# LariWa/Fractal-Image-Compression

Hardware: AMD Instinct MI355X
Metric: range-block matches/sec (8x8 R, 16x16 D, 8 iso) (higher is better)
Workload: dtype u8

## Files before the change

### fractal-image-compression_amd/csrc/fic_capi.cpp

```cpp
#include "fic_internal.h"

namespace ficd {

thread_local std::string g_err;
thread_local int g_err_code = 0;

int fail(int code, const char* fmt, ...)
{
    char buf[512];
    va_list ap;
    va_start(ap, fmt);
    vsnprintf(buf, sizeof(buf), fmt, ap);
    va_end(ap);
    g_err = buf;
    g_err_code = code;
    return code;
}

int check_device(int device)
{
    int ndev = fic_device_count();
    if (ndev <= 0 || device < 0 || device >= ndev) return fail(FIC_E_NO_DEVICE, "no HIP device %d (this library has no CPU path)", device);
    HIP_TRY(hipSetDevice(device));
    return FIC_OK;
// ... 357 lines not shown
{
    const FicGeom& g = c->g;
    const QShape q = q_shape(g);
    const int tsz = 64 * g.NR;
    const int cpr = fic_q_cols_per_range(g.B, g.n_iso);
    const int ct_begin = tile0 * tsz * cpr / 32, ct_end = tile1 * tsz * cpr / 32;
    int nchunks = c->opt_chunks;
    if (nchunks <= 0) {
        const long long base_wg = (long long)((ct_end - ct_begin + q.CT - 1) / q.CT) * g.planes;
        const long long resident = 256LL * fic_q_resident(g.B);
        auto ceil_div = [](long long a, long long b) { return (a + b - 1) / b; };
        const long long min_tiles = g.n_iso == 8 ? 30 : 14;
        long long fill = base_wg < resident ? ceil_div(2 * resident, base_wg) : 1;
        if (fill > q.ndtiles / min_tiles) fill = q.ndtiles / min_tiles;
        long long bal = ceil_div(8 * resident, base_wg);
        if (bal > q.ndtiles / 1024) bal = q.ndtiles / 1024;
        const long long nc = fill > bal ? fill : bal;
        nchunks = (int)(nc < 1 ? 1 : nc);
    }
    if (nchunks > q.ndtiles) nchunks = q.ndtiles;
    int tiles_per_chunk = (q.ndtiles + nchunks - 1) / nchunks;
    tiles_per_chunk = (tiles_per_chunk + q.unroll - 1) / q.unroll * q.unroll;
    nchunks = (q.ndtiles + tiles_per_chunk - 1) / tiles_per_chunk;
    if (fused_fin && !c->q_fin) {
        const size_t nfin = (size_t)g.planes * (q.nct_alloc / q.CT + 1);
        HIP_TRY(hipMalloc((void**)&c->q_fin, nfin * sizeof(unsigned int)));
        HIP_TRY(hipMemsetAsync(c->q_fin, 0, nfin * sizeof(unsigned int), s));
    }
    if (fic_launch_sweep_q(c->b, c->q_pool, c->q_flat, c->q_rng, c->q_rngC, c->q_E, c->q_thg, g, ct_begin, ct_end, q.ndtiles, q.ndtiles_alloc,
                           q.nct_alloc, tiles_per_chunk, nchunks, s, c->q_stats, c->opt_noflag, fused_fin ? &c->o : nullptr, c->q_fin,
                           r_begin, r_count))
        return fail(FIC_E_HIP, "k_sweep_q launch failed");
    *nchunks_out = nchunks;
    c->last_tiles_per_chunk = tiles_per_chunk;
    return FIC_OK;
}

}

extern "C" {

#ifdef FIC_BUILD_XCHECK
const char* fic_version(void) { return "fic-hip 0.3 (gfx950, +xcheck sweeps)"; }
#else
const char* fic_version(void) { return "fic-hip 0.3 (gfx950)"; }
#endif
const char* fic_last_error(void) { return g_err.c_str(); }
int fic_last_error_code(void) { return g_err_code; }

int fic_device_count(void)
{
    int n = 0;
    if (hipGetDeviceCount(&n) != hipSuccess) return 0;
    return n;
// ... 153 lines not shown
        const char* env = getenv("FIC_SWEEP");
        if (env && env[0] >= '2' && env[0] <= '6' && env[1] == '\0' && g.full) {
            const int want = env[0] - '0';
            kind = want == 5 ? valu : want;
        }
    }
    if (kind >= 2 && !g.full) return fail(FIC_E_ARGUMENT, "fast sweep needs full search (wK == Dw == Dh)");
#ifndef FIC_BUILD_XCHECK
    if (kind == 3 || kind == 4) return fail(FIC_E_ARGUMENT, "sweep %d (cross-check kernel) is not in this build (FIC_BUILD_XCHECK=0)", kind);
#endif
    if (kind == 5 && !d4_available(g)) return fail(FIC_E_ARGUMENT, "sweep 5 (k_sweep_d4) needs full search, n_iso = 8 and B = 8");
    if (kind == 6 && g.Nd >= (1 << 24)) return fail(FIC_E_ARGUMENT, "sweep 6 (k_sweep_q) needs a pool of fewer than 2^24 blocks");
    const int tsz = 64 * g.NR;
    const int tile0 = range_begin / tsz;
    const int tile1 = (range_begin + range_count + tsz - 1) / tsz;
    const int ntiles = tile1 - tile0;
    int nchunks = 1;
    int rc = FIC_OK;
    bool fused_prep = false;
    if (kind == 6) {
        const QShape q = q_shape(g);
        fused_prep = fic_q_prep_fused(g, q.ndtiles_alloc, tile1 * (64 * g.NR) / 64 - tile0 * (64 * g.NR) / 64) != 0;
    }
    if (!fused_prep && fic_launch_scale(c->b.gray, c->b.scaled, g, s)) return fail(FIC_E_HIP, "k_scale launch failed");
    if (kind == 6) {
        rc = q_prep(c, tile0, tile1, s);
    } else {
        if (fic_launch_pool(c->b.scaled, c->b.pool_pix, c->b.pool_st, c->b.pool_var, c->b.pool_s64, g, s))
            return fail(FIC_E_HIP, "k_pool launch failed");
        if (kind != 5 && !c->b.rng_pix) {
            int rca = dev_alloc(&c->b.rng_pix, (size_t)g.planes * g.Nr_pad * g.n_iso * g.DW);
            if (rca) return rca;
        }
        if (fic_launch_range(c->b.gray, c->b.rng_pix, c->b.rng_st, g, s, kind == 5 ? 0 : 1)) return fail(FIC_E_HIP, "k_range launch failed");
        HIP_TRY(hipMemset2DAsync(c->b.key + (size_t)tile0 * tsz, (size_t)g.Nr_pad * sizeof(unsigned long long), 0xFF,
                                 (size_t)ntiles * tsz * sizeof(unsigned long long), (size_t)g.planes, s));
        if (kind == 5) rc = d4_prep(c, s);
        else if (kind >= 3) rc = matrix_core_prep(c, kind, s);
    }
    if (rc == FIC_OK) rc = time_begin(c, s);
    if (rc == FIC_OK) {
        if (kind == 1) {
            if (fic_launch_sweep_generic(c->b, g, range_begin, range_count, s)) rc = fail(FIC_E_HIP, "k_sweep_generic launch failed");
        } else if (kind == 6) {
            rc = q_sweep(c, tile0, tile1, s, &nchunks, fused_prep, range_begin, range_count);
        } else if (kind == 5) {
            rc = d4_sweep(c, tile0, tile1 - tile0, s, &nchunks);
        } else if (kind >= 3) {
            rc = matrix_core_sweep(c, kind, tile0, tile1, s, &nchunks);
        } else {
            rc = valu_sweep(c, tile0, tile1 - tile0, s, &nchunks);
        }
    }
    if (rc == FIC_OK) rc = time_end(c, s);
    if (rc != FIC_OK) return rc;
    c->last_chunks = nchunks;
    c->last_kind = kind;
    c->last_fused = fused_prep ? 1 : 0;
    if (!fused_prep &&
        fic_launch_finalize(c->b, c->o, g, range_begin, range_count, s, (kind == 5 || kind == 6) ? 1 : 0)) return fail(FIC_E_HIP, "k_finalize launch failed");
    c->encoded_any = true;
    return FIC_OK;
}

int fic_ctx_sync(fic_ctx* c)
{
    if (!c) return fail(FIC_E_ARGUMENT, "fic_ctx_sync: null context");
    HIP_TRY(hipSetDevice(c->device));
    HIP_TRY(hipStreamSynchronize(c->last_stream));
    return FIC_OK;
}

int fic_ctx_get_results_host(fic_ctx* c, int32_t* idx_local, float* a, float* b, int32_t* iso, int32_t* qrows,
                             int32_t* idx_global, float* err)
{
    if (!c) return fail(FIC_E_ARGUMENT, "fic_ctx_get_results_host: null context");
    if (!c->encoded_any) return fail(FIC_E_STATE, "fic_ctx_get_results_host: nothing encoded yet");
    HIP_TRY(hipSetDevice(c->device));
    HIP_TRY(hipStreamSynchronize(c->last_stream));
    size_t n = (size_t)c->g.planes * c->g.Nr;
    if (n > (size_t)65536) {
        if (idx_local) HIP_TRY(hipMemcpy(idx_local, c->o.idx_local, n * 4, hipMemcpyDeviceToHost));
// ... 281 lines not shown
```

### fractal-image-compression_amd/csrc/fic_q.hip

```cpp
#include <hip/hip_runtime.h>
#include <stdint.h>
#include <math.h>
#include <string.h>
#include <stdlib.h>
#include <type_traits>
#include "fic_device.h"
#include "fic_launch.h"
#include "fic_devfn.h"

typedef int v4i __attribute__((ext_vector_type(4)));
typedef float v16f __attribute__((ext_vector_type(16)));
typedef _Float16 f16x8 __attribute__((ext_vector_type(8)));

#define FIC_Q_LEVEL 0.99999237060546875f
#define FIC_Q_TAU_ALL 3.0e38f
#define FIC_Q_TAU_NONE (-1.0f)
#define FIC_Q_LMIN 0.26f
#define FIC_Q_ECOEF 7.0e-4f
#define FIC_Q_EABS 1.6e-5f
#define FIC_Q_QCAP 1280
#define FIC_Q_QFLUSH 256

#ifndef FIC_Q_CTW_B8
#define FIC_Q_CTW_B8 4
// ... 62 lines not shown
        const int i = t / B, ry = t % B;
        const int d = dtile * 32 + i;
        uint32_t w[B / 4];
#pragma unroll
        for (int q = 0; q < B / 4; q++) w[q] = 0u;
        if (d < g.Nd) {
            const int c = d % g.Dw, r = d / g.Dw;
            const size_t so = (size_t)plane * g.Ws * g.Hs + (size_t)(r * g.abstand + ry) * g.Ws + c * g.abstand;
            if constexpr (!FUSE) {
                __builtin_memcpy(w, scaled_in + so, B);
            } else {
                const int ys = r * g.abstand + ry, xs0 = c * g.abstand;
                const uint8_t* im = gray + (size_t)plane * g.W * g.H + (size_t)(2 * ys) * g.W + 2 * xs0;
                uint32_t top[B / 2], bot[B / 2];
                __builtin_memcpy(top, im, 2 * B);
                __builtin_memcpy(bot, im + g.W, 2 * B);
#pragma unroll
                for (int x = 0; x < B; x++) {
                    const uint32_t t2 = top[x >> 1] >> (16 * (x & 1)), b2 = bot[x >> 1] >> (16 * (x & 1));
                    const int tap4 = (2 * (xs0 + x) + 1 >= g.H) ? 128 : (int)((b2 >> 8) & 0xffu);
                    const int m = (int)(t2 & 0xffu) + (int)((t2 >> 8) & 0xffu) + (int)(b2 & 0xffu) + tap4;
                    w[x >> 2] |= (uint32_t)(m / 4) << (8 * (x & 3));
                }
                __builtin_memcpy(scaled_out + so, w, B);
            }
        }
        uint32_t sum = 0, sq = 0;
#pragma unroll
        for (int q = 0; q < B / 4; q++) {
            sum = __builtin_amdgcn_sad_u8(w[q], 0u, sum);
            sq = __builtin_amdgcn_udot4(w[q], w[q], sq, false);
            *(uint32_t*)&pix[i][ry * B + 4 * q] = w[q];
        }
        s_sum[i][ry] = (int)sum;
        s_sq[i][ry] = (int)sq;
    }
    __syncthreads();
    for (int t = threadIdx.x; t < 32 * n / 16; t += 256) {
        const int i = t / (n / 16), q = t % (n / 16);
        const int d = dtile * 32 + i;
        if (d < g.Nd) *(uint4*)(pool_pix + ((size_t)plane * g.Nd_pad + d) * n + 16 * q) = *(const uint4*)&pix[i][16 * q];
    }
    if (threadIdx.x < 32) {
        const int i = threadIdx.x, d = dtile * 32 + i;
        int S = 0, Q = 0;
        for (int t = 0; t < B; t++) { S += s_sum[i][t]; Q += s_sq[i][t]; }
        const int m = S >> g.lgn;
// ... 30 lines not shown
            for (int u = 0; u < 8; u++) px[u] = (int)(((u < 4 ? pw.x : pw.y) >> (8 * (u & 3))) & 0xffu);
#pragma unroll
            for (int u = 0; u < 4; u++)
                v[u] = f16_pair(__fmul_rn((float)(px[2 * u] - dM), w), __fmul_rn((float)(px[2 * u + 1] - dM), w));
        } else {
            const bool odd = m >= NK / 2;
            const int p0 = 16 * (odd ? m - NK / 2 : m) + 8 * h;
            const uint2 pw = *(const uint2*)&pix[i][p0], qw = *(const uint2*)&pix[i][n - 8 - p0];
            float f[8];
#pragma unroll
            for (int u = 0; u < 8; u++) {
                const int a = (int)(((u < 4 ? pw.x : pw.y) >> (8 * (u & 3))) & 0xffu);
                const int b = (int)(((u < 4 ? qw.y : qw.x) >> (8 * (3 - (u & 3)))) & 0xffu);
                f[u] = __fmul_rn(__fmul_rn((float)(odd ? a - b : a + b - 2 * dM), w), 0.5f);
            }
#pragma unroll
            for (int u = 0; u < 4; u++) v[u] = f16_pair(f[2 * u], f[2 * u + 1]);
        }
        poolQ[((size_t)plane * ndtiles_alloc + dtile) * NK * 64 + t] = v;
    }
    if (threadIdx.x == 0) dflat[(size_t)plane * ndtiles_alloc + dtile] = s_nonflat ? 0u : 1u;
}
template <int B>
__global__ __launch_bounds__(256) void k_pool_q(const uint8_t* __restrict__ scaled, uint8_t* __restrict__ pool_pix,
                                                FicDomStat* __restrict__ pool_st, uint32_t* __restrict__ pool_var,
                                                double* __restrict__ pool_s64, v4i* __restrict__ poolQ,
                                                uint32_t* __restrict__ dflat, FicGeom g, int ndtiles_alloc, int folded, int shape16)
{
    pool_q_body<B, false>(blockIdx.x, blockIdx.y, scaled, nullptr, nullptr, pool_pix, pool_st, pool_var, pool_s64, poolQ, dflat, g,
                          ndtiles_alloc, folded, shape16);
}

__global__ __launch_bounds__(256) void k_range_q(const uint8_t* __restrict__ gray, FicRngStat* __restrict__ rng_st,
                                                 float* __restrict__ rngE, unsigned long long* __restrict__ key,
                                                 uint32_t* __restrict__ theta_g, v4i* __restrict__ rngQ,
                                                 uint32_t* __restrict__ rngC, FicGeom g, int nct_alloc, int grp0, int mode,
                                                 int staged, int shape16)
{
    __shared__ __attribute__((aligned(16))) uint8_t blk[64 * (256 + 4)];
    extern __shared__ __attribute__((aligned(16))) uint8_t cpy[];
    __shared__ int s_rM[64];
    const int plane = blockIdx.y;
    const int grp = grp0 + blockIdx.x;
    const int B = g.B, n = g.n, DW = g.DW, NK = n / 16;
    const int lgB = B == 4 ? 2 : (B == 8 ? 3 : 4);
    const int stride = n + 4;
    const int j0 = grp * 64;
    const uint8_t* img = gray + (size_t)plane * g.W * g.H;
    for (int i = threadIdx.x; i < 64 * DW; i += 256) {
        const int l = i / DW, wd = i % DW;
        const int j = j0 + l;
        uint32_t v = 0;
        if (j < g.Nr) {
// ... 330 lines not shown
}
__device__ __forceinline__ float max16_sum(const v16f& a, const v16f& b)
{
    float v[16];
#pragma unroll
    for (int e = 0; e < 16; e++) v[e] = fabsf(a[e]) + fabsf(b[e]);
    const float m0 = fmaxf(fmaxf(v[0], v[1]), v[2]), m1 = fmaxf(fmaxf(v[3], v[4]), v[5]), m2 = fmaxf(fmaxf(v[6], v[7]), v[8]);
    const float m3 = fmaxf(fmaxf(v[9], v[10]), v[11]), m4 = fmaxf(fmaxf(v[12], v[13]), v[14]);
    return fmaxf(fmaxf(fmaxf(m0, m1), m2), fmaxf(fmaxf(m3, m4), v[15]));
}

template <int MODE> struct QMode {
    static constexpr int CSHIFT = (MODE == 0 || MODE == 3) ? 0 : ((MODE == 1 || MODE == 4) ? 3 : 2);
    static constexpr int NISO = (MODE == 0 || MODE == 3) ? 1 : 8;
    static constexpr bool RGB = MODE == 3 || MODE == 4;
};
template <int MODE> __device__ __forceinline__ int q_col_iso(int c) { return MODE == 2 ? (c == 0 ? 0 : (c == 1 ? 1 : (c == 2 ? 4 : 6))) : c; }

__device__ __forceinline__ void q_key_min(unsigned long long* keyp, unsigned long long best)
{
    if (best < __hip_atomic_load(keyp, __ATOMIC_RELAXED, __HIP_MEMORY_SCOPE_AGENT)) atomicMin(keyp, best);
}

template <int NK, int MODE>
__device__ __forceinline__ void q_flush(const QArgs& A, const uint32_t* myq, int qn, int plane, int ctw0, int lane)
{
    constexpr int NISO = QMode<MODE>::NISO, CSHIFT = QMode<MODE>::CSHIFT;
    constexpr int B = NK == 1 ? 4 : (NK == 4 ? 8 : 16);
    const FicRngStat* rst = A.rng_st + (size_t)plane * A.Nr_pad;
    const double* p64 = A.pool_s64 + (size_t)plane * A.Nd_pad;
    const FicDomStat* pst = A.pool_st + (size_t)plane * A.Nd_pad;
    unsigned long long* keyp = A.key + (size_t)plane * A.Nr_pad;
    const uint32_t* cop = A.rngC + (size_t)plane * A.Nr_pad * (1 << CSHIFT) * (A.n / 4);
    for (int base = 0; base < qn; base += 64) {
        const int i = base + lane;
        if (i < qn) {
            const uint32_t ent = myq[i];
            const uint32_t d = ent & 0x00FFFFFFu;
            if (d >= (uint32_t)A.Nd) continue;
            const int col = ctw0 * 32 + (int)(ent >> 24);
            if constexpr (MODE == 4) {
                const int j = col >> 3, k = col & 7;
                const FicRngStat rs = rst[j];
                const FicRgbDomStat ds = A.rgb_dst[d];
                const int16_t* rt = A.rgb_rng + (size_t)j * (B * B);
                const uint16_t* ps = A.rgb_pool + (size_t)d * (B * B);
                int ax, bx, cx, ay, by, cy;
                iso_affine(k, B - 1, ax, bx, cx, ay, by, cy);
                const int ox = ay * B + ax, oy = by * B + bx, o0 = cy * B + cx;
// ... 15 lines not shown
                const FicRgbDomStat ds = A.rgb_dst[d];
                const uint4* rt = (const uint4*)(A.rgb_rng + (size_t)col * (B * B));
                const uint4* ps = (const uint4*)(A.rgb_pool + (size_t)d * (B * B));
                float kov = 0.0f;
#pragma unroll 4
                for (int q = 0; q < B * B / 8; q++) {
                    const uint4 r4 = rt[q], p4 = ps[q];
                    const uint32_t rw[4] = {r4.x, r4.y, r4.z, r4.w}, pw[4] = {p4.x, p4.y, p4.z, p4.w};
#pragma unroll
                    for (int u = 0; u < 4; u++) {
                        kov = __fadd_rn(kov, (float)((int)(int16_t)(rw[u] & 0xffffu) * ((int)(pw[u] & 0xffffu) - ds.msum)));
                        kov = __fadd_rn(kov, (float)((int)(int16_t)(rw[u] >> 16) * ((int)(pw[u] >> 16) - ds.msum)));
                    }
                }
                const float vRf = (float)rs.rem;
                float r = (rs.rem == 0 || ds.vD == 0) ? 0.0f : __fdiv_rn(kov, __fmul_rn(vRf, (float)ds.vD));
                r = __fmul_rn(r, r);
                const float e = __fmul_rn(__fmul_rn(vRf, vRf), __fsub_rn(1.0f, r));
                q_key_min(&keyp[col], ((unsigned long long)f32_orderable(e) << 32) | d);
                continue;
            }
            const int j = col >> CSHIFT, k = q_col_iso<MODE>(col & ((1 << CSHIFT) - 1));
            const int k2 = k == 0 ? 2 : (k == 1 ? 3 : k + 1);
            const unsigned long long cur = __hip_atomic_load(&keyp[j], __ATOMIC_RELAXED, __HIP_MEMORY_SCOPE_AGENT);
            const FicRngStat rs = rst[j];
            const int Sd = (int)pst[d].sum;
            const double s64 = p64[d];
            const uint4* cw = (const uint4*)(cop + (size_t)col * (B * B / 4));
            const uint4* dw = (const uint4*)(A.pool_pix + ((size_t)plane * A.Nd_pad + d) * A.n);
            uint32_t s = 0, s2 = 0;
#pragma unroll
            for (int q = 0; q < B * B / 16; q++) {
                const uint4 c4 = cw[q], d4 = dw[q];
                s = __builtin_amdgcn_udot4(c4.x, d4.x, s, false);
                s = __builtin_amdgcn_udot4(c4.y, d4.y, s, false);
                s = __builtin_amdgcn_udot4(c4.z, d4.z, s, false);
                s = __builtin_amdgcn_udot4(c4.w, d4.w, s, false);
                if constexpr (MODE == 2) {
                    const uint4 m4 = dw[B * B / 16 - 1 - q];
                    s2 = __builtin_amdgcn_udot4(c4.x, __builtin_bswap32(m4.w), s2, false);
                    s2 = __builtin_amdgcn_udot4(c4.y, __builtin_bswap32(m4.z), s2, false);
                    s2 = __builtin_amdgcn_udot4(c4.z, __builtin_bswap32(m4.y), s2, false);
                    s2 = __builtin_amdgcn_udot4(c4.w, __builtin_bswap32(m4.x), s2, false);
                }
            }
            const int base_c = rs.rM * Sd + (Sd >> A.lgn) * rs.rem;
            const float err = exact_error((int)s - base_c, rs.rem, s64);
            unsigned long long best = ((unsigned long long)f32_orderable(err) << 32) | (d * (uint32_t)NISO + (uint32_t)k);
            if constexpr (MODE == 2) {
                const float err2 = exact_error((int)s2 - base_c, rs.rem, s64);
                const unsigned long long b2 = ((unsigned long long)f32_orderable(err2) << 32) | (d * (uint32_t)NISO + (uint32_t)k2);
                best = b2 < best ? b2 : best;
            }
            if (best < cur) atomicMin(&keyp[j], best);
        }
    }
}

template <int MODE, bool SEED = false>
__device__ __forceinline__ float q_share_max(float v)
{
    if constexpr (QMode<MODE>::CSHIFT >= 2) {
        v = fmaxf(v, __uint_as_float((uint32_t)__builtin_amdgcn_update_dpp(0, (int)__float_as_uint(v), 0xB1, 0xF, 0xF, true)));
        v = fmaxf(v, __uint_as_float((uint32_t)__builtin_amdgcn_update_dpp(0, (int)__float_as_uint(v), 0x4E, 0xF, 0xF, true)));
    }
    if constexpr (QMode<MODE>::CSHIFT == 3)
        v = fmaxf(v, __uint_as_float((uint32_t)__builtin_amdgcn_update_dpp(0, (int)__float_as_uint(v), 0x141, 0xF, 0xF, true)));
    if constexpr (SEED) {
        const int partner = (int)((threadIdx.x & 63u) ^ 32u) << 2;
        return fmaxf(v, __int_as_float(__builtin_amdgcn_ds_bpermute(partner, __float_as_int(v))));
    } else {
        const uint32_t u = __float_as_uint(v);
        const auto r = __builtin_amdgcn_permlane32_swap(u, u, false, false);
        return fmaxf(__uint_as_float(r[0]), __uint_as_float(r[1]));
    }
}

template <int NK, int MODE>
// ... 25 lines not shown
            const unsigned long long none = FIC_KEY_NONE;
            asm volatile("global_atomic_umin_x2 %0, %1, %2, off sc0\n\ts_waitcnt vmcnt(0)"
                         : "=&v"(kk) : "v"(A.key + (size_t)plane * A.Nr_pad + j), "v"(none) : "memory");
            const uint32_t c = (uint32_t)kk;
            const int wloc = (int)(c / (uint32_t)NISO), k = (int)(c % (uint32_t)NISO);
            const int gi = wloc;
            const uint32_t* pp = (const uint32_t*)(A.pool_pix + ((size_t)plane * A.Nd_pad + gi) * A.n);
            const uint8_t* blk = A.gray + (size_t)plane * g.W * g.H + (size_t)((j / g.Rw) * B) * g.W + (j % g.Rw) * B;
            uint32_t acc = 0, s2;
            iso_dot<B, false>(blk, g.W, k, pp, acc, s2);
            finalize_store(A.out, g, plane, j, kk, wloc, gi, k, acc, A.pool_st[(size_t)plane * A.Nd_pad + gi],
                           A.rng_st[(size_t)plane * A.Nr_pad + j], A.pool_var[(size_t)plane * A.Nd_pad + gi]);
        }
    }
}

template <int NK, int MODE, bool MULTI, bool GFAST>
__device__ __forceinline__ void sweep_q_body(const QArgs& A)
{
    constexpr int CTW = fic_q_ctw(NK), CT = FIC_Q_WPG * CTW;
    constexpr int CSHIFT = QMode<MODE>::CSHIFT;
    constexpr bool FOLD = MODE == 2;
    constexpr int NKA = FOLD ? NK / 2 : NK;
    __shared__ uint32_t sQ[FIC_Q_WPG][FIC_Q_QCAP + 4];
    const int lane = threadIdx.x & 63;
    const int wave = __builtin_amdgcn_readfirstlane(threadIdx.x >> 6);
    int combo_, gx_;
    xcd_decode(blockIdx.x, A.nchunks * A.planes, A.nctg, combo_, gx_);
    const int plane = combo_ / A.nchunks;
    const int chunk = combo_ % A.nchunks;
    const int ctw0 = A.ct_begin + gx_ * CT + wave * CTW;
    const int dt0 = chunk * A.tiles_per_chunk;
    int dt1 = dt0 + A.tiles_per_chunk;
    if (dt1 > A.ndtiles_loop) dt1 = A.ndtiles_loop;
    __shared__ int s_wdone;
    if (dt0 >= A.ndtiles || ctw0 >= A.ct_end) {
        if (A.fin_count) q_finalize_tail<NK, MODE>(A, plane, gx_, &s_wdone, lane);
        return;
    }
    const unsigned long long clk0 = A.stats ? clock64() : 0ull, tick0 = A.stats ? wall_clock64() : 0ull;
    int nci = A.ct_end - ctw0;
    if (nci > CTW) nci = CTW;

    const int jcol = lane & 31, half = lane >> 5;
    const FicRngStat* rst = A.rng_st + (size_t)plane * A.Nr_pad;
    uint32_t* const thg = A.theta_g + (size_t)plane * A.Nr_pad;
    uint32_t* const myq = sQ[wave];
    uint32_t* const myqn = myq + FIC_Q_QCAP;
    const uint32_t myqn_lds = (uint32_t)(uintptr_t)(__attribute__((address_space(3))) uint32_t*)myqn;
    if (lane == 0) *myqn = 0u;

    v4i rb[CTW][NK];
    {
        const v4i* rp = A.rngQ + ((size_t)plane * A.nct_alloc + ctw0) * NK * 64 + lane;
#pragma unroll
        for (int ci = 0; ci < CTW; ci++)
#pragma unroll
            for (int m = 0; m < NK; m++) rb[ci][m] = rp[(ci * NK + m) * 64];
    }
    float tau[CTW], E[CTW], lmn[CTW];
    float gl[GFAST ? CTW : 1];
#pragma unroll
    for (int ci = 0; ci < (GFAST ? CTW : 1); ci++) gl[ci] = -1.0f;
    uint32_t okbits = 0, raise = 0;
#pragma unroll
    for (int ci = 0; ci < CTW; ci++) {
        const int col = (ctw0 + ci) * 32 + jcol;
        const int j = col >> CSHIFT;
        const bool ok = j < A.Nr && ci < nci;
        const int rem = ok ? rst[j].rem : 0;
        E[ci] = ok ? A.rngE[(size_t)plane * A.Nr_pad + j] : 0.0f;
        tau[ci] = (ok && rem != 0 && !A.dbg_noflag) ? FIC_Q_TAU_NONE : FIC_Q_TAU_ALL;
        lmn[ci] = FIC_Q_LMIN * (float)rem;
        okbits |= ok ? 1u << ci : 0u;
        raise |= (ok && rem != 0) ? 1u << ci : 0u;
    }

    const v4i* pa = A.poolQ + (size_t)plane * A.ndtiles_alloc * NK * 64 + lane;
    const uint32_t AS4* pflat = (const uint32_t AS4*)(uintptr_t)(A.dflat + (size_t)plane * A.ndtiles_alloc);
    const v16f zero = {0, 0, 0, 0, 0, 0, 0, 0, 0, 0, 0, 0, 0, 0, 0, 0};
    int qn = 0;
    unsigned st_slow = 0, st_pairs = 0;

    auto flush = [&]() __attribute__((always_inline)) {
        q_flush<NK, MODE>(A, myq, qn, plane, ctw0, lane);
        qn = 0;
        if (lane == 0) *myqn = 0u;
        __builtin_amdgcn_s_waitcnt(0x0F70);
    };
    auto val = [&](const v16f& acc, const v16f& acc2, int e) __attribute__((always_inline)) {
        return FOLD ? fabsf(acc[e]) + fabsf(acc2[e]) : fabsf(acc[e]);
    };
    auto slow_tile = [&](const v16f& acc, const v16f& acc2, float mx, int ci, int dt, bool first) __attribute__((always_inline)) {
        if (!first && __builtin_amdgcn_ballot_w64(mx > 0.0f) == 0 && pflat[dt] != 0u) return;
        st_slow++;
        const bool ok = (okbits >> ci) & 1u;
        const bool mayraise = (raise >> ci) & 1u;
        const int colw = ci * 32 + jcol;
        const int jg = ((ctw0 + ci) * 32 + jcol) >> CSHIFT;
        const uint32_t g = (MULTI && !GFAST && mayraise) ? thg[jg] : FIC_Q_THG_NONE;
        const uint32_t ent0 = (uint32_t)(dt * 32 + 4 * half) | ((uint32_t)colw << 24);
        if (first) {
            const float lo = __fsub_rn(q_share_max<MODE>(ok ? mx : 0.0f), E[ci]);
            if (mayraise && lo >= lmn[ci]) tau[ci] = fmaxf(tau[ci], __fsub_rn(__fmul_rn(lo, FIC_Q_LEVEL), E[ci]));
        }
        const bool cand0 = first && dt == 0 && half == 0 && ok && (jcol & ((1 << CSHIFT) - 1)) == 0;
        uint32_t hm = 0;
#pragma unroll
// ... 133 lines not shown
    if (A.stats && lane == 0 && (blockIdx.x & 15) == 0 && wave == 0) {
        atomicAdd(&A.stats[0], ph1 - clk0);
        atomicAdd(&A.stats[1], ph2 - ph1);
        atomicAdd(&A.stats[2], (unsigned long long)clock64() - ph2);
        atomicAdd(&A.stats[4], (unsigned long long)(clock64() - clk0));
        atomicAdd(&A.stats[5], (unsigned long long)(wall_clock64() - tick0));
        atomicAdd(&A.stats[6], 1ull);
        atomicAdd(&A.stats[3], (unsigned long long)st_slow);
        atomicAdd(&A.stats[7], (unsigned long long)st_pairs);
    }
    if (false)
#endif
    if (A.stats && lane == 0) {
        atomicAdd(&A.stats[0], (unsigned long long)(dt1 - dt0) * (unsigned)nci);
        atomicAdd(&A.stats[1], (unsigned long long)st_slow);
        atomicAdd(&A.stats[2], (unsigned long long)st_pairs);
        atomicAdd(&A.stats[3], 1ull);
        if ((blockIdx.x & 15) == 0 && wave == 0) {
            atomicAdd(&A.stats[4], (unsigned long long)(clock64() - clk0));
            atomicAdd(&A.stats[5], (unsigned long long)(wall_clock64() - tick0));
            atomicAdd(&A.stats[6], 1ull);
        }
    }
    if (A.fin_count) q_finalize_tail<NK, MODE>(A, plane, gx_, &s_wdone, lane);
}

typedef float v4f __attribute__((ext_vector_type(4)));
__device__ __forceinline__ v4f mfma16_f16(v4i a, v4i b, v4f c)
{
    return __builtin_amdgcn_mfma_f32_16x16x32_f16(__builtin_bit_cast(f16x8, a), __builtin_bit_cast(f16x8, b), c, 0, 0, 0);
}
__device__ __forceinline__ float max8_abs(const v4f& x0, const v4f& x1)
{
    const float m0 = max3f(fabsf(x0[0]), fabsf(x0[1]), fabsf(x0[2])), m1 = max3f(fabsf(x0[3]), fabsf(x1[0]), fabsf(x1[1]));
    return max3f(m0, m1, max3f(fabsf(x1[2]), fabsf(x1[3]), 0.0f));
}
template <bool SEED = false>
__device__ __forceinline__ float q16_share_max(float v)
{
    const int partner = (int)((threadIdx.x & 63u) ^ 16u) << 2;
    const float w = fmaxf(v, __int_as_float(__builtin_amdgcn_ds_bpermute(partner, __float_as_int(v))));
    if constexpr (SEED) return fmaxf(w, __int_as_float(__builtin_amdgcn_ds_bpermute((int)((threadIdx.x & 63u) ^ 32u) << 2, __float_as_int(w))));
    const uint32_t uw = __float_as_uint(w);
    const auto q = __builtin_amdgcn_permlane32_swap(uw, uw, false, false);
    return fmaxf(__uint_as_float(q[0]), __uint_as_float(q[1]));
}
template <int NK, bool MULTI, bool GFAST>
__device__ __forceinline__ void sweep_q16_body(const QArgs& A)
{
    constexpr int CTW = fic_q_ctw(NK), CT = FIC_Q_WPG * CTW, CU = 2 * CTW, KS = NK / 2;
    __shared__ uint32_t sQ[FIC_Q_WPG][FIC_Q_QCAP + 4];
    const int lane = threadIdx.x & 63;
    const int wave = __builtin_amdgcn_readfirstlane(threadIdx.x >> 6);
    int combo_, gx_;
    xcd_decode(blockIdx.x, A.nchunks * A.planes, A.nctg, combo_, gx_);
    const int plane = combo_ / A.nchunks;
    const int chunk = combo_ % A.nchunks;
    const int ctw0 = A.ct_begin + gx_ * CT + wave * CTW;
    const int dt0 = chunk * A.tiles_per_chunk;
    int dt1 = dt0 + A.tiles_per_chunk;
    if (dt1 > A.ndtiles_loop) dt1 = A.ndtiles_loop;
    __shared__ int s_wdone;
    if (dt0 >= A.ndtiles || ctw0 >= A.ct_end) {
        if (A.fin_count) q_finalize_tail<NK, 0>(A, plane, gx_, &s_wdone, lane);
        return;
    }
    const unsigned long long clk0 = A.stats ? clock64() : 0ull, tick0 = A.stats ? wall_clock64() : 0ull;
    int nci = A.ct_end - ctw0;
    if (nci > CTW) nci = CTW;

    const int c16 = lane & 15, g4 = lane >> 4;
    const FicRngStat* rst = A.rng_st + (size_t)plane * A.Nr_pad;
    uint32_t* const thg = A.theta_g + (size_t)plane * A.Nr_pad;
    uint32_t* const myq = sQ[wave];
    uint32_t* const myqn = myq + FIC_Q_QCAP;
    const uint32_t myqn_lds = (uint32_t)(uintptr_t)(__attribute__((address_space(3))) uint32_t*)myqn;
    if (lane == 0) *myqn = 0u;

    v4i rb[CTW][NK];
    {
        const v4i* rp = A.rngQ + ((size_t)plane * A.nct_alloc + ctw0) * NK * 64 + lane;
#pragma unroll
        for (int ci = 0; ci < CTW; ci++)
#pragma unroll
            for (int m = 0; m < NK; m++) rb[ci][m] = rp[(ci * NK + m) * 64];
    }
    float tau[CU], E[CU], lmn[CU];
    float gl[GFAST ? CU : 1];
#pragma unroll
    for (int cj = 0; cj < (GFAST ? CU : 1); cj++) gl[cj] = -1.0f;
    uint32_t okbits = 0, raise = 0;
#pragma unroll
    for (int cj = 0; cj < CU; cj++) {
        const int j = ctw0 * 32 + cj * 16 + c16;
        const bool ok = j < A.Nr && (cj >> 1) < nci;
        const int rem = ok ? rst[j].rem : 0;
        E[cj] = ok ? A.rngE[(size_t)plane * A.Nr_pad + j] : 0.0f;
        tau[cj] = (ok && rem != 0 && !A.dbg_noflag) ? FIC_Q_TAU_NONE : FIC_Q_TAU_ALL;
        lmn[cj] = FIC_Q_LMIN * (float)rem;
        okbits |= ok ? 1u << cj : 0u;
        raise |= (ok && rem != 0) ? 1u << cj : 0u;
    }
    const v4i* pa = A.poolQ + (size_t)plane * A.ndtiles_alloc * NK * 64 + lane;
    const uint32_t AS4* pflat = (const uint32_t AS4*)(uintptr_t)(A.dflat + (size_t)plane * A.ndtiles_alloc);
    const v4f zero = {0, 0, 0, 0};
    int qn = 0;
    unsigned st_slow = 0, st_pairs = 0;

    auto flush = [&]() __attribute__((always_inline)) {
        q_flush<NK, 0>(A, myq, qn, plane, ctw0, lane);
        qn = 0;
        if (lane == 0) *myqn = 0u;
        __builtin_amdgcn_s_waitcnt(0x0F70);
    };
    auto val = [&](const v4f& x0, const v4f& x1, int e) __attribute__((always_inline)) { return fabsf(e < 4 ? x0[e] : x1[e - 4]); };
    auto slow_unit = [&](const v4f& x0, const v4f& x1, float mx, int cj, int dt, bool first) __attribute__((always_inline)) {
        if (!first && __builtin_amdgcn_ballot_w64(mx > 0.0f) == 0 && pflat[dt] != 0u) return;
        st_slow++;
        const bool ok = (okbits >> cj) & 1u;
        const bool mayraise = (raise >> cj) & 1u;
        const int colw = cj * 16 + c16;
        const int jg = ctw0 * 32 + colw;
        const uint32_t g = (MULTI && !GFAST && mayraise) ? thg[jg] : FIC_Q_THG_NONE;
        const uint32_t ent0 = (uint32_t)(dt * 32 + 4 * g4) | ((uint32_t)colw << 24);
        if (first) {
            const float lo = __fsub_rn(q16_share_max<>(ok ? mx : 0.0f), E[cj]);
            if (mayraise && lo >= lmn[cj]) tau[cj] = fmaxf(tau[cj], __fsub_rn(__fmul_rn(lo, FIC_Q_LEVEL), E[cj]));
        }
        const bool cand0 = first && dt == 0 && g4 == 0 && ok;
        uint32_t hm = 0;
#pragma unroll
        for (int e = 7; e >= 0; e--)
            hm = __builtin_amdgcn_alignbit(hm, __float_as_uint(__fsub_rn(tau[cj], val(x0, x1, e))), 31);
// ... 77 lines not shown
            const float mx = max8_abs(x0, x1);
            const bool hit = mx > tau[cj];
            if (__builtin_expect((__builtin_amdgcn_ballot_w64(hit) != 0) | first, 0)) slow_unit(x0, x1, mx, cj, dt, first);
            x0 = n0;
            x1 = n1;
        }
    };
    for (int dt = dt0; dt < dt1; dt += 2) {
        step(dt, a0, a1, dt == dt0, std::integral_constant<int, 0>());
        step(dt + 1, a1, a0, false, std::integral_constant<int, 1>());
    }
    flush();
    if (A.stats && lane == 0) {
        atomicAdd(&A.stats[0], (unsigned long long)(dt1 - dt0) * (unsigned)nci);
        atomicAdd(&A.stats[1], (unsigned long long)st_slow);
        atomicAdd(&A.stats[2], (unsigned long long)st_pairs);
        atomicAdd(&A.stats[3], 1ull);
        if ((blockIdx.x & 15) == 0 && wave == 0) {
            atomicAdd(&A.stats[4], (unsigned long long)(clock64() - clk0));
            atomicAdd(&A.stats[5], (unsigned long long)(wall_clock64() - tick0));
            atomicAdd(&A.stats[6], 1ull);
        }
    }
    if (A.fin_count) q_finalize_tail<NK, 0>(A, plane, gx_, &s_wdone, lane);
}

template <int NK, int MODE, bool MULTI>
__global__ __launch_bounds__(64 * FIC_Q_WPG, NK == 4 ? FIC_Q_WAVES_B8 : (NK < 4 ? FIC_Q_WAVES_B4 : 1)) void k_sweep_q(QArgs A)
{
    sweep_q_body<NK, MODE, MULTI, false>(A);
}
template <int NK, int MODE>
__global__ __launch_bounds__(64 * FIC_Q_WPG, NK == 4 ? FIC_Q_WAVES_B8 : (NK < 4 ? FIC_Q_WAVES_B4 : 1)) void k_sweep_qs(QArgs A)
{
    sweep_q_body<NK, MODE, true, true>(A);
}
template <int NK, bool MULTI>
__global__ __launch_bounds__(64 * FIC_Q_WPG, NK == 4 ? FIC_Q_WAVES_B8 : 1) void k_sweep_q16(QArgs A)
{
    sweep_q16_body<NK, MULTI, false>(A);
}
template <int NK>
__global__ __launch_bounds__(64 * FIC_Q_WPG, NK == 4 ? FIC_Q_WAVES_B8 : 1) void k_sweep_q16s(QArgs A)
{
    sweep_q16_body<NK, true, true>(A);
}

// ... 37 lines not shown
int fic_q_unroll(int B, int n_iso) { (void)B; (void)n_iso; return FIC_Q_UNROLL; }
int fic_q_shape16(const FicGeom& g)
{
    const long long ndtiles = (g.Nd + 31) / 32;
    int want = g.q_shape;
    if (want == 0) {
        const char* env = getenv("FIC_Q_SHAPE");
        if (env && (env[0] == '1' || env[0] == '2') && env[1] == '\0') want = env[0] - '0';
    }
    if (!FIC_Q_SHAPE16 || g.n_iso != 1 || g.B < 8 || want == 2) return 0;
    return (want == 1 || ndtiles * (g.n / 16) >= 100000) ? 1 : 0;
}
int fic_q_resident(int B) { return (B == 4 ? FIC_Q_WAVES_B4 : (B == 8 ? FIC_Q_WAVES_B8 : 1)) * 4 / FIC_Q_WPG; }

int fic_q_prep_fused(const FicGeom& g, int ndtiles_alloc, int ngrp)
{
    return (g.B == 8 && (long long)g.planes * (ndtiles_alloc + ngrp) <= 1024) ? 1 : 0;
}
int fic_launch_q_prep(const FicBuffers& b, void* poolQ, void* dflat, void* rngQ, void* rngC, void* rngE, void* theta_g,
                      const FicGeom& g, int ndtiles_alloc, int nct_alloc, int grp0, int ngrp, hipStream_t s)
{
    const int mode = fic_q_mode(g.B, g.n_iso);
    const int shape16 = fic_q_shape16(g);
    if (fic_q_prep_fused(g, ndtiles_alloc, ngrp)) {
        auto pk = mode == 0 ? k_prep_q8<0> : k_prep_q8<2>;
        hipLaunchKernelGGL(pk, dim3(ndtiles_alloc + ngrp, g.planes), dim3(256), 0, s, (const uint8_t*)b.gray, b.scaled, b.pool_pix, b.pool_st,
                           b.pool_var, b.pool_s64, (v4i*)poolQ, (uint32_t*)dflat, b.rng_st, (float*)rngE, b.key, (uint32_t*)theta_g,
                           (v4i*)rngQ, (uint32_t*)rngC, g, ndtiles_alloc, nct_alloc, grp0, shape16);
        FIC_LAUNCH_CHECK();
        return 0;
    }
    auto pool = g.B == 4 ? k_pool_q<4> : (g.B == 8 ? k_pool_q<8> : k_pool_q<16>);
    hipLaunchKernelGGL(pool, dim3(ndtiles_alloc, g.planes), dim3(256), 0, s, (const uint8_t*)b.scaled, b.pool_pix,
                       b.pool_st, b.pool_var, b.pool_s64, (v4i*)poolQ, (uint32_t*)dflat, g, ndtiles_alloc, mode == 2 ? 1 : 0, shape16);
    FIC_LAUNCH_CHECK();
    const size_t stage_bytes = (size_t)64 * fic_q_cols_per_range(g.B, g.n_iso) * (g.n + 8);
    const int staged = stage_bytes <= 40 * 1024 ? 1 : 0;
    if (g.B == 8 && mode != 1) {
        auto rk = mode == 0 ? k_range_q8<0> : k_range_q8<2>;
        hipLaunchKernelGGL(rk, dim3(ngrp, g.planes), dim3(256), 0, s, (const uint8_t*)b.gray, b.rng_st, (float*)rngE, b.key,
                           (uint32_t*)theta_g, (v4i*)rngQ, (uint32_t*)rngC, g, nct_alloc, grp0, shape16);
    } else {
        hipLaunchKernelGGL(k_range_q, dim3(ngrp, g.planes), dim3(256), staged ? stage_bytes : 0, s, (const uint8_t*)b.gray, b.rng_st,
                           (float*)rngE, b.key, (uint32_t*)theta_g, (v4i*)rngQ, (uint32_t*)rngC, g, nct_alloc, grp0, mode, staged, shape16);
    }
    FIC_LAUNCH_CHECK();
    return 0;
}

int fic_launch_sweep_q(const FicBuffers& b, const void* poolQ, const void* dflat, const void* rngQ, const void* rngC, const void* rngE,
                       void* theta_g, const FicGeom& g, int ct_begin, int ct_end, int ndtiles, int ndtiles_alloc,
                       int nct_alloc, int tiles_per_chunk, int nchunks, hipStream_t s, unsigned long long* stats, int dbg_noflag,
                       const FicOutputs* fin_out, unsigned int* fin_count, int r_begin, int r_count)
{
    QArgs A;
    A.stats = stats;
    A.dbg_noflag = dbg_noflag;
    A.fin_count = fin_out ? fin_count : nullptr;
    if (fin_out) A.out = *fin_out; else memset(&A.out, 0, sizeof(A.out));
    A.geom = g; A.gray = b.gray; A.pool_var = b.pool_var; A.r_begin = r_begin; A.r_end = r_begin + r_count;
    A.poolQ = (const v4i*)poolQ; A.dflat = (const uint32_t*)dflat; A.pool_pix = b.pool_pix; A.pool_st = b.pool_st;
    A.pool_s64 = b.pool_s64; A.rngQ = (const v4i*)rngQ; A.rngC = (const uint32_t*)rngC; A.rng_st = b.rng_st;
    A.rngE = (const float*)rngE; A.key = b.key; A.theta_g = (uint32_t*)theta_g;
    A.Nd = g.Nd; A.Nd_pad = g.Nd_pad; A.Nr = g.Nr; A.Nr_pad = g.Nr_pad; A.n = g.n; A.lgn = g.lgn; A.W = g.W; A.H = g.H; A.Rw = g.Rw;
    const int unroll = fic_q_unroll(g.B, g.n_iso);
    A.ndtiles = ndtiles; A.ndtiles_loop = (ndtiles + unroll - 1) / unroll * unroll; A.ndtiles_alloc = ndtiles_alloc; A.nct_alloc = nct_alloc;
    A.ct_begin = ct_begin; A.ct_end = ct_end; A.tiles_per_chunk = tiles_per_chunk; A.nchunks = nchunks;
    const int CT = fic_q_ct(g.B);
    A.nctg = (ct_end - ct_begin + CT - 1) / CT;
    A.planes = g.planes;
    A.rgb_rng = nullptr; A.rgb_pool = nullptr; A.rgb_dst = nullptr;
    if (ct_begin + A.nctg * CT > nct_alloc || g.Nd >= (1 << 24) || A.ndtiles_loop + unroll > ndtiles_alloc || tiles_per_chunk % unroll)
        return (int)hipErrorInvalidValue;
    dim3 grid((unsigned)(nchunks * g.planes) * (unsigned)A.nctg), block(64 * FIC_Q_WPG);
    const int mode = fic_q_mode(g.B, g.n_iso);
    if (!q_launch(g.B * g.B / 16, mode, fic_q_multi_kind(nchunks, tiles_per_chunk), grid, block, s, A, fic_q_shape16(g))) return (int)hipErrorInvalidValue;
    FIC_LAUNCH_CHECK();
    return 0;
}

__global__ __launch_bounds__(256) void k_pool_qrgb(const uint16_t* __restrict__ pool_sum, const FicRgbDomStat* __restrict__ dst,
// ... 135 lines not shown
```

Baseline: 135.1 million.

## Fuse downscale into pool kernel and keep per-wave LDS keys for single-chunk sweeps

The separate k_scale launch is dropped for the q sweep, and the unfused pool kernel now downsamples from the gray image itself, writing only the scaled pixels it owns. When the sweep runs as a single chunk on grey modes, each wave keeps its best-match keys in LDS using workgroup-scope atomic min instead of global atomics. It then finalizes its own ranges in-kernel, so the separate finalize launch is skipped. This removes two kernel launches and global atomic traffic, at the cost of extra LDS per workgroup and a new geometry precondition on stride and pool shape.

```diff
diff --git a/fractal-image-compression_amd/csrc/fic_capi.cpp b/fractal-image-compression_amd/csrc/fic_capi.cpp
--- a/fractal-image-compression_amd/csrc/fic_capi.cpp
+++ b/fractal-image-compression_amd/csrc/fic_capi.cpp
@@ -403,14 +403,14 @@
     int tiles_per_chunk = (q.ndtiles + nchunks - 1) / nchunks;
     tiles_per_chunk = (tiles_per_chunk + q.unroll - 1) / q.unroll * q.unroll;
     nchunks = (q.ndtiles + tiles_per_chunk - 1) / tiles_per_chunk;
-    if (fused_fin && !c->q_fin) {
+    if (fused_fin && nchunks > 1 && !c->q_fin) {
         const size_t nfin = (size_t)g.planes * (q.nct_alloc / q.CT + 1);
         HIP_TRY(hipMalloc((void**)&c->q_fin, nfin * sizeof(unsigned int)));
         HIP_TRY(hipMemsetAsync(c->q_fin, 0, nfin * sizeof(unsigned int), s));
     }
     if (fic_launch_sweep_q(c->b, c->q_pool, c->q_flat, c->q_rng, c->q_rngC, c->q_E, c->q_thg, g, ct_begin, ct_end, q.ndtiles, q.ndtiles_alloc,
-                           q.nct_alloc, tiles_per_chunk, nchunks, s, c->q_stats, c->opt_noflag, fused_fin ? &c->o : nullptr, c->q_fin,
-                           r_begin, r_count))
+                           q.nct_alloc, tiles_per_chunk, nchunks, s, c->q_stats, c->opt_noflag, (fused_fin || nchunks == 1) ? &c->o : nullptr,
+                           c->q_fin, r_begin, r_count))
         return fail(FIC_E_HIP, "k_sweep_q launch failed");
     *nchunks_out = nchunks;
     c->last_tiles_per_chunk = tiles_per_chunk;
@@ -610,7 +610,7 @@
         const QShape q = q_shape(g);
         fused_prep = fic_q_prep_fused(g, q.ndtiles_alloc, tile1 * (64 * g.NR) / 64 - tile0 * (64 * g.NR) / 64) != 0;
     }
-    if (!fused_prep && fic_launch_scale(c->b.gray, c->b.scaled, g, s)) return fail(FIC_E_HIP, "k_scale launch failed");
+    if (kind != 6 && fic_launch_scale(c->b.gray, c->b.scaled, g, s)) return fail(FIC_E_HIP, "k_scale launch failed");
     if (kind == 6) {
         rc = q_prep(c, tile0, tile1, s);
     } else {
@@ -645,7 +645,8 @@
     c->last_chunks = nchunks;
     c->last_kind = kind;
     c->last_fused = fused_prep ? 1 : 0;
-    if (!fused_prep &&
+    const bool sweep_finalised = fused_prep || (kind == 6 && nchunks == 1);
+    if (!sweep_finalised &&
         fic_launch_finalize(c->b, c->o, g, range_begin, range_count, s, (kind == 5 || kind == 6) ? 1 : 0)) return fail(FIC_E_HIP, "k_finalize launch failed");
     c->encoded_any = true;
     return FIC_OK;
diff --git a/fractal-image-compression_amd/csrc/fic_q.hip b/fractal-image-compression_amd/csrc/fic_q.hip
--- a/fractal-image-compression_amd/csrc/fic_q.hip
+++ b/fractal-image-compression_amd/csrc/fic_q.hip
@@ -108,7 +108,11 @@
                     const int m = (int)(t2 & 0xffu) + (int)((t2 >> 8) & 0xffu) + (int)(b2 & 0xffu) + tap4;
                     w[x >> 2] |= (uint32_t)(m / 4) << (8 * (x & 3));
                 }
-                __builtin_memcpy(scaled_out + so, w, B);
+                constexpr int AB = B / 4;
+                if (ry < AB || r == g.Dh - 1) {
+                    if (c == g.Dw - 1) __builtin_memcpy(scaled_out + so, w, B);
+                    else __builtin_memcpy(scaled_out + so, w, AB);
+                }
             }
         }
         uint32_t sum = 0, sq = 0;
@@ -185,13 +189,13 @@
     if (threadIdx.x == 0) dflat[(size_t)plane * ndtiles_alloc + dtile] = s_nonflat ? 0u : 1u;
 }
 template <int B>
-__global__ __launch_bounds__(256) void k_pool_q(const uint8_t* __restrict__ scaled, uint8_t* __restrict__ pool_pix,
+__global__ __launch_bounds__(256) void k_pool_q(const uint8_t* __restrict__ gray, uint8_t* __restrict__ scaled, uint8_t* __restrict__ pool_pix,
                                                 FicDomStat* __restrict__ pool_st, uint32_t* __restrict__ pool_var,
                                                 double* __restrict__ pool_s64, v4i* __restrict__ poolQ,
                                                 uint32_t* __restrict__ dflat, FicGeom g, int ndtiles_alloc, int folded, int shape16)
 {
-    pool_q_body<B, false>(blockIdx.x, blockIdx.y, scaled, nullptr, nullptr, pool_pix, pool_st, pool_var, pool_s64, poolQ, dflat, g,
-                          ndtiles_alloc, folded, shape16);
+    pool_q_body<B, true>(blockIdx.x, blockIdx.y, nullptr, gray, scaled, pool_pix, pool_st, pool_var, pool_s64, poolQ, dflat, g,
+                         ndtiles_alloc, folded, shape16);
 }
 
 __global__ __launch_bounds__(256) void k_range_q(const uint8_t* __restrict__ gray, FicRngStat* __restrict__ rng_st,
@@ -568,9 +572,14 @@
     if (best < __hip_atomic_load(keyp, __ATOMIC_RELAXED, __HIP_MEMORY_SCOPE_AGENT)) atomicMin(keyp, best);
 }
 
-template <int NK, int MODE>
-__device__ __forceinline__ void q_flush(const QArgs& A, const uint32_t* myq, int qn, int plane, int ctw0, int lane)
-{
+template <int MODE, bool MULTI> struct QOwn {
+    static constexpr bool value = !MULTI && !QMode<MODE>::RGB;
+};
+template <int NK, int MODE, bool OWN = false>
+__device__ __forceinline__ void q_flush(const QArgs& A, const uint32_t* myq, int qn, int plane, int ctw0, int lane,
+                                        unsigned long long* lk = nullptr)
+{
+    static_assert(!(OWN && QMode<MODE>::RGB), "wave-owned keys: grey modes only");
     constexpr int NISO = QMode<MODE>::NISO, CSHIFT = QMode<MODE>::CSHIFT;
     constexpr int B = NK == 1 ? 4 : (NK == 4 ? 8 : 16);
     const FicRngStat* rst = A.rng_st + (size_t)plane * A.Nr_pad;
@@ -632,7 +641,8 @@
             }
             const int j = col >> CSHIFT, k = q_col_iso<MODE>(col & ((1 << CSHIFT) - 1));
             const int k2 = k == 0 ? 2 : (k == 1 ? 3 : k + 1);
-            const unsigned long long cur = __hip_atomic_load(&keyp[j], __ATOMIC_RELAXED, __HIP_MEMORY_SCOPE_AGENT);
+            unsigned long long cur = 0ull;
+            if constexpr (!OWN) cur = __hip_atomic_load(&keyp[j], __ATOMIC_RELAXED, __HIP_MEMORY_SCOPE_AGENT);
             const FicRngStat rs = rst[j];
             const int Sd = (int)pst[d].sum;
             const double s64 = p64[d];
@@ -662,8 +672,36 @@
                 const unsigned long long b2 = ((unsigned long long)f32_orderable(err2) << 32) | (d * (uint32_t)NISO + (uint32_t)k2);
                 best = b2 < best ? b2 : best;
             }
-            if (best < cur) atomicMin(&keyp[j], best);
-        }
+            if constexpr (OWN) {
+                __hip_atomic_fetch_min((__attribute__((address_space(3))) unsigned long long*)(lk + (j - ((ctw0 * 32) >> CSHIFT))), best,
+                                       __ATOMIC_RELAXED, __HIP_MEMORY_SCOPE_WORKGROUP);
+            } else {
+                if (best < cur) atomicMin(&keyp[j], best);
+            }
+        }
+    }
+}
+
+template <int NK, int MODE>
+__device__ __forceinline__ void q_finalize_own(const QArgs& A, int plane, int ctw0, int nci, const unsigned long long* lk, int lane)
+{
+    constexpr int CSHIFT = QMode<MODE>::CSHIFT, NISO = QMode<MODE>::NISO;
+    constexpr int B = NK == 1 ? 4 : (NK == 4 ? 8 : 16);
+    const FicGeom& g = A.geom;
+    const int j0 = (ctw0 * 32) >> CSHIFT, nj = (nci * 32) >> CSHIFT;
+    for (int jj = lane; jj < nj; jj += 64) {
+        const int j = j0 + jj;
+        if (j < A.r_begin || j >= A.r_end) continue;
+        const unsigned long long kk = lk[jj];
+        const uint32_t c = (uint32_t)kk;
+        const int wloc = (int)(c / (uint32_t)NISO), k = (int)(c % (uint32_t)NISO);
+        const int gi = wloc;
+        const uint32_t* pp = (const uint32_t*)(A.pool_pix + ((size_t)plane * A.Nd_pad + gi) * A.n);
+        const uint8_t* blk = A.gray + (size_t)plane * g.W * g.H + (size_t)((j / g.Rw) * B) * g.W + (j % g.Rw) * B;
+        uint32_t acc = 0, s2;
+        iso_dot<B, false>(blk, g.W, k, pp, acc, s2);
+        finalize_store(A.out, g, plane, j, kk, wloc, gi, k, acc, A.pool_st[(size_t)plane * A.Nd_pad + gi],
+                       A.rng_st[(size_t)plane * A.Nr_pad + j], A.pool_var[(size_t)plane * A.Nd_pad + gi]);
     }
 }
 
@@ -735,7 +773,10 @@
     constexpr int CSHIFT = QMode<MODE>::CSHIFT;
     constexpr bool FOLD = MODE == 2;
     constexpr int NKA = FOLD ? NK / 2 : NK;
+    constexpr bool OWN = QOwn<MODE, MULTI>::value;
+    constexpr int NOWN = (CTW * 32) >> CSHIFT;
     __shared__ uint32_t sQ[FIC_Q_WPG][FIC_Q_QCAP + 4];
+    __shared__ unsigned long long sK[OWN ? FIC_Q_WPG : 1][OWN ? NOWN : 1];
     const int lane = threadIdx.x & 63;
     const int wave = __builtin_amdgcn_readfirstlane(threadIdx.x >> 6);
     int combo_, gx_;
@@ -748,12 +789,20 @@
     if (dt1 > A.ndtiles_loop) dt1 = A.ndtiles_loop;
     __shared__ int s_wdone;
     if (dt0 >= A.ndtiles || ctw0 >= A.ct_end) {
-        if (A.fin_count) q_finalize_tail<NK, MODE>(A, plane, gx_, &s_wdone, lane);
+        if constexpr (!OWN) {
+            if (A.fin_count) q_finalize_tail<NK, MODE>(A, plane, gx_, &s_wdone, lane);
+        }
         return;
     }
     const unsigned long long clk0 = A.stats ? clock64() : 0ull, tick0 = A.stats ? wall_clock64() : 0ull;
     int nci = A.ct_end - ctw0;
     if (nci > CTW) nci = CTW;
+    unsigned long long* const myk = sK[OWN ? wave : 0];
+    if constexpr (OWN) {
+#pragma unroll
+        for (int jj = 0; jj < NOWN; jj += 64)
+            if (jj + lane < NOWN) myk[jj + lane] = FIC_KEY_NONE;
+    }
 
     const int jcol = lane & 31, half = lane >> 5;
     const FicRngStat* rst = A.rng_st + (size_t)plane * A.Nr_pad;
@@ -796,7 +845,7 @@
     unsigned st_slow = 0, st_pairs = 0;
 
     auto flush = [&]() __attribute__((always_inline)) {
-        q_flush<NK, MODE>(A, myq, qn, plane, ctw0, lane);
+        q_flush<NK, MODE, OWN>(A, myq, qn, plane, ctw0, lane, myk);
         qn = 0;
         if (lane == 0) *myqn = 0u;
         __builtin_amdgcn_s_waitcnt(0x0F70);
@@ -976,7 +1025,8 @@
             atomicAdd(&A.stats[6], 1ull);
         }
     }
-    if (A.fin_count) q_finalize_tail<NK, MODE>(A, plane, gx_, &s_wdone, lane);
+    if constexpr (OWN) q_finalize_own<NK, MODE>(A, plane, ctw0, nci, myk, lane);
+    else if (A.fin_count) q_finalize_tail<NK, MODE>(A, plane, gx_, &s_wdone, lane);
 }
 
 typedef float v4f __attribute__((ext_vector_type(4)));
@@ -1003,7 +1053,10 @@
 __device__ __forceinline__ void sweep_q16_body(const QArgs& A)
 {
     constexpr int CTW = fic_q_ctw(NK), CT = FIC_Q_WPG * CTW, CU = 2 * CTW, KS = NK / 2;
+    constexpr bool OWN = QOwn<0, MULTI>::value;
+    constexpr int NOWN = CTW * 32;
     __shared__ uint32_t sQ[FIC_Q_WPG][FIC_Q_QCAP + 4];
+    __shared__ unsigned long long sK[OWN ? FIC_Q_WPG : 1][OWN ? NOWN : 1];
     const int lane = threadIdx.x & 63;
     const int wave = __builtin_amdgcn_readfirstlane(threadIdx.x >> 6);
     int combo_, gx_;
@@ -1016,12 +1069,20 @@
     if (dt1 > A.ndtiles_loop) dt1 = A.ndtiles_loop;
     __shared__ int s_wdone;
     if (dt0 >= A.ndtiles || ctw0 >= A.ct_end) {
-        if (A.fin_count) q_finalize_tail<NK, 0>(A, plane, gx_, &s_wdone, lane);
+        if constexpr (!OWN) {
+            if (A.fin_count) q_finalize_tail<NK, 0>(A, plane, gx_, &s_wdone, lane);
+        }
         return;
     }
     const unsigned long long clk0 = A.stats ? clock64() : 0ull, tick0 = A.stats ? wall_clock64() : 0ull;
     int nci = A.ct_end - ctw0;
     if (nci > CTW) nci = CTW;
+    unsigned long long* const myk = sK[OWN ? wave : 0];
+    if constexpr (OWN) {
+#pragma unroll
+        for (int jj = 0; jj < NOWN; jj += 64)
+            if (jj + lane < NOWN) myk[jj + lane] = FIC_KEY_NONE;
+    }
 
     const int c16 = lane & 15, g4 = lane >> 4;
     const FicRngStat* rst = A.rng_st + (size_t)plane * A.Nr_pad;
@@ -1062,7 +1123,7 @@
     unsigned st_slow = 0, st_pairs = 0;
 
     auto flush = [&]() __attribute__((always_inline)) {
-        q_flush<NK, 0>(A, myq, qn, plane, ctw0, lane);
+        q_flush<NK, 0, OWN>(A, myq, qn, plane, ctw0, lane, myk);
         qn = 0;
         if (lane == 0) *myqn = 0u;
         __builtin_amdgcn_s_waitcnt(0x0F70);
@@ -1186,7 +1247,8 @@
             atomicAdd(&A.stats[6], 1ull);
         }
     }
-    if (A.fin_count) q_finalize_tail<NK, 0>(A, plane, gx_, &s_wdone, lane);
+    if constexpr (OWN) q_finalize_own<NK, 0>(A, plane, ctw0, nci, myk, lane);
+    else if (A.fin_count) q_finalize_tail<NK, 0>(A, plane, gx_, &s_wdone, lane);
 }
 
 template <int NK, int MODE, bool MULTI>
@@ -1270,6 +1332,7 @@
 {
     const int mode = fic_q_mode(g.B, g.n_iso);
     const int shape16 = fic_q_shape16(g);
+    if (g.abstand * 4 != g.B || (g.Dw - 1) * g.abstand + g.B != g.Ws || (g.Dh - 1) * g.abstand + g.B != g.Hs) return (int)hipErrorInvalidValue;
     if (fic_q_prep_fused(g, ndtiles_alloc, ngrp)) {
         auto pk = mode == 0 ? k_prep_q8<0> : k_prep_q8<2>;
         hipLaunchKernelGGL(pk, dim3(ndtiles_alloc + ngrp, g.planes), dim3(256), 0, s, (const uint8_t*)b.gray, b.scaled, b.pool_pix, b.pool_st,
@@ -1279,7 +1342,7 @@
         return 0;
     }
     auto pool = g.B == 4 ? k_pool_q<4> : (g.B == 8 ? k_pool_q<8> : k_pool_q<16>);
-    hipLaunchKernelGGL(pool, dim3(ndtiles_alloc, g.planes), dim3(256), 0, s, (const uint8_t*)b.scaled, b.pool_pix,
+    hipLaunchKernelGGL(pool, dim3(ndtiles_alloc, g.planes), dim3(256), 0, s, (const uint8_t*)b.gray, b.scaled, b.pool_pix,
                        b.pool_st, b.pool_var, b.pool_s64, (v4i*)poolQ, (uint32_t*)dflat, g, ndtiles_alloc, mode == 2 ? 1 : 0, shape16);
     FIC_LAUNCH_CHECK();
     const size_t stage_bytes = (size_t)64 * fic_q_cols_per_range(g.B, g.n_iso) * (g.n + 8);
@@ -1304,7 +1367,8 @@
     QArgs A;
     A.stats = stats;
     A.dbg_noflag = dbg_noflag;
-    A.fin_count = fin_out ? fin_count : nullptr;
+    if (nchunks <= 1 && !fin_out) return (int)hipErrorInvalidValue;
+    A.fin_count = (fin_out && nchunks > 1) ? fin_count : nullptr;
     if (fin_out) A.out = *fin_out; else memset(&A.out, 0, sizeof(A.out));
     A.geom = g; A.gray = b.gray; A.pool_var = b.pool_var; A.r_begin = r_begin; A.r_end = r_begin + r_count;
     A.poolQ = (const v4i*)poolQ; A.dflat = (const uint32_t*)dflat; A.pool_pix = b.pool_pix; A.pool_st = b.pool_st;
```

Measured after the change: 137.6 million, median of 6. 1.9% higher.
